# hjr37/diff-gaussian-rasterization

Hardware: AMD Instinct MI355X
Metric: Mviews/sec fwd+bwd @1080p, 500k Gaussians (higher is better)
Workload: dtype f32

## Files before the change

diff-gaussian-rasterization_amd/csrc/dgr_common.h:

```cpp
#pragma once
#include <hip/hip_runtime.h>
#include <stdint.h>

#define DGR_BLOCK_X 16
#define DGR_BLOCK_Y 16
#define DGR_TILE_PIX 256
#define DGR_NEAR 0.2f
#define DGR_TAG_SHIFT 28
#define DGR_ID_MASK ((1u << DGR_TAG_SHIFT) - 1u)
#ifndef DGR_COUNT_STRIDE
#define DGR_COUNT_STRIDE 16
#endif

#define DGR_SCHED_CLASSES 32

namespace dgr {

__host__ __device__ inline size_t align_up(size_t x, size_t a) { return (x + a - 1) / a * a; }

__device__ inline uint32_t sched_class(uint32_t n) {
    if (n == 0u) return 0u;
    const uint32_t l = 31u - (uint32_t)__clz((int)n);
    const uint32_t half = l ? (n >> (l - 1u)) & 1u : 0u;
    const uint32_t c = 1u + 2u * l + half;
    return c < (uint32_t)DGR_SCHED_CLASSES - 1u ? c : (uint32_t)DGR_SCHED_CLASSES - 1u;
}

#ifndef DGR_REC_STRIDE
#define DGR_REC_STRIDE 4
#endif
struct GeometryView {
    float4* rec;
    float* depths;
    int* radii;
    ushort4* rect;
    uint8_t* clamped;
    uint32_t* goff;
    uint32_t* block_tiles;
    float4* shd;
    size_t bytes;
};
__host__ __device__ inline GeometryView carve_geometry(char* base, int P) {
    GeometryView g;
    size_t o = 0;
    g.rec = (float4*)(base + o);      o = align_up(o + sizeof(float4) * DGR_REC_STRIDE * (size_t)P, 256);
    g.depths = (float*)(base + o);    o = align_up(o + sizeof(float) * (size_t)P, 256);
    g.radii = (int*)(base + o);       o = align_up(o + sizeof(int) * (size_t)P, 256);
    g.rect = (ushort4*)(base + o);    o = align_up(o + sizeof(ushort4) * (size_t)P, 256);
    g.clamped = (uint8_t*)(base + o); o = align_up(o + (size_t)P, 256);
    g.goff = (uint32_t*)(base + o);   o = align_up(o + sizeof(uint32_t) * (size_t)P, 256);
    g.block_tiles = (uint32_t*)(base + o); o = align_up(o + sizeof(uint32_t) * (((size_t)P + 255) / 256), 256);
    g.shd = (float4*)(base + o);      o = align_up(o + sizeof(float4) * 3 * (size_t)P, 256);
    g.bytes = o;
    return g;
}

enum { BLEND_SCHEDULE = 1, BLEND_LISTS_QUADRANT = 4, BLEND_LISTS_AUTO = 8 };
enum { BLEND_FLAG_SCHEDULE = 1, BLEND_FLAG_OVERFLOWED = 2, BLEND_FLAG_QUADRANT_LISTS = 4 };

struct ImageView {
    int* status;
    uint32_t* cursor;
    uint32_t* tile_count;
    uint2* ranges;
    uint4* tile_sched;
    uint32_t* n_contrib;
    float* final_T;
    uint32_t* n_valid;
    uint32_t* first_contrib;
    size_t bytes;
};
__host__ __device__ inline int tiles_x(int W) { return (W + DGR_BLOCK_X - 1) / DGR_BLOCK_X; }
__host__ __device__ inline int tiles_y(int H) { return (H + DGR_BLOCK_Y - 1) / DGR_BLOCK_Y; }
__host__ __device__ inline ImageView carve_image(char* base, int W, int H) {
    ImageView v;
    const size_t tiles = (size_t)tiles_x(W) * tiles_y(H), N = (size_t)W * H;
    size_t o = 0;
    v.status = (int*)(base + o);
    v.cursor = (uint32_t*)(base + o + 64);  o = align_up(o + 4 * sizeof(int), 256);
    v.tile_count = (uint32_t*)(base + o); o = align_up(o + tiles * 4 * DGR_COUNT_STRIDE, 256);
    v.ranges = (uint2*)(base + o);        o = align_up(o + tiles * 8, 256);
    v.tile_sched = (uint4*)(base + o);    o = align_up(o + tiles * 16, 256);
    v.n_contrib = (uint32_t*)(base + o);  o = align_up(o + N * 4, 256);
    v.final_T = (float*)(base + o);       o = align_up(o + N * 4, 256);
    v.n_valid = (uint32_t*)(base + o);    o = align_up(o + N * 4, 256);
// ... 113 lines not shown
```

diff-gaussian-rasterization_amd/csrc/gaussian_math.h:

```cpp
#pragma once
#include "dgr_common.h"

#pragma clang fp contract(off)

namespace dgr {
namespace {

struct M3 {
    float m[3][3];
};
__device__ __forceinline__ M3 mul(const M3& A, const M3& B) {
    M3 R;
#pragma unroll
    for (int c = 0; c < 3; c++)
#pragma unroll
        for (int r = 0; r < 3; r++) R.m[c][r] = A.m[0][r] * B.m[c][0] + A.m[1][r] * B.m[c][1] + A.m[2][r] * B.m[c][2];
    return R;
}
__device__ __forceinline__ M3 transpose(const M3& A) {
    M3 R;
#pragma unroll
    for (int c = 0; c < 3; c++)
#pragma unroll
        for (int r = 0; r < 3; r++) R.m[c][r] = A.m[r][c];
// ... 127 lines not shown
    const M3 S = diag3(mod * sc.x, mod * sc.y, mod * sc.z);
    const M3 Mm = mul(S, R);
    const M3 Sigma = mul(transpose(Mm), Mm);
    c3[0] = Sigma.m[0][0]; c3[1] = Sigma.m[0][1]; c3[2] = Sigma.m[0][2];
    c3[3] = Sigma.m[1][1]; c3[4] = Sigma.m[1][2]; c3[5] = Sigma.m[2][2];
}
template <class Args>
__device__ __forceinline__ void load_cov3d(const Args& a, int idx, float (&c3)[6]) {
    if (a.cov3D_precomp) {
        const float* c3p = a.cov3D_precomp + 6 * (size_t)idx;
#pragma unroll
        for (int i = 0; i < 6; i++) c3[i] = c3p[i];
    } else {
        compute_cov3d(a.scales, a.rotations, a.scale_modifier, idx, c3);
    }
}

}

constexpr int SHT_ROWS = 32, SHT_LD = 52;
__device__ __forceinline__ void wave_sync() {
    __builtin_amdgcn_fence(__ATOMIC_ACQ_REL, "wavefront");
    __builtin_amdgcn_wave_barrier();
}
__device__ __forceinline__ void store_streaming(float4* dst, float4 v) {
    typedef float v4f __attribute__((ext_vector_type(4)));
    __builtin_nontemporal_store(v4f{v.x, v.y, v.z, v.w}, reinterpret_cast<v4f*>(dst));
}
__device__ __forceinline__ float4 load_streaming(const float4* src) {
    typedef float v4f __attribute__((ext_vector_type(4)));
    const v4f v = __builtin_nontemporal_load(reinterpret_cast<const v4f*>(src));
    return make_float4(v.x, v.y, v.z, v.w);
}
__device__ __forceinline__ void sh_rows_to_lanes(const float* __restrict__ src, size_t g_block, float* lds, float (&f)[48]) {
    const int wave = threadIdx.x >> 6, lane = threadIdx.x & 63;
    float* my = lds + wave * (SHT_ROWS * SHT_LD);
    const float4* base = reinterpret_cast<const float4*>(src) + (g_block + (size_t)wave * 64) * 12;
#pragma unroll
    for (int r = 0; r < 2; r++) {
        const float4* p = base + (size_t)r * SHT_ROWS * 12;
#pragma unroll
        for (int i = 0; i < 6; i++) {
            const int e = i * 64 + lane;
            const int g = e / 12, c = e - 12 * g;
            *reinterpret_cast<float4*>(my + g * SHT_LD + 4 * c) = load_streaming(p + e);
        }
        wave_sync();
        if ((lane >> 5) == r) {
            const float* row = my + (lane & 31) * SHT_LD;
#pragma unroll
            for (int c = 0; c < 12; c++) {
                const float4 v = *reinterpret_cast<const float4*>(row + 4 * c);
                f[4 * c] = v.x; f[4 * c + 1] = v.y; f[4 * c + 2] = v.z; f[4 * c + 3] = v.w;
            }
        }
        wave_sync();
    }
}
__device__ __forceinline__ void lanes_to_sh_rows(const float (&f)[48], float* __restrict__ dst, size_t g_block, float* lds) {
    const int wave = threadIdx.x >> 6, lane = threadIdx.x & 63;
    float* my = lds + wave * (SHT_ROWS * SHT_LD);
    float4* base = reinterpret_cast<float4*>(dst) + (g_block + (size_t)wave * 64) * 12;
#pragma unroll
    for (int r = 0; r < 2; r++) {
        if ((lane >> 5) == r) {
            float* row = my + (lane & 31) * SHT_LD;
#pragma unroll
            for (int c = 0; c < 12; c++)
                *reinterpret_cast<float4*>(row + 4 * c) = make_float4(f[4 * c], f[4 * c + 1], f[4 * c + 2], f[4 * c + 3]);
        }
        wave_sync();
        float4* p = base + (size_t)r * SHT_ROWS * 12;
#pragma unroll
        for (int i = 0; i < 6; i++) {
            const int e = i * 64 + lane;
            const int g = e / 12, c = e - 12 * g;
            store_streaming(p + e, *reinterpret_cast<const float4*>(my + g * SHT_LD + 4 * c));
        }
        wave_sync();
    }
}
// ... 88 lines not shown
```

diff-gaussian-rasterization_amd/csrc/preprocess_bwd.hip:

```cpp
#include "dgr_common.h"
#include <algorithm>

#include "kernels.h"
#include "gaussian_math.h"
#include "pose_reduce.h"

#pragma clang fp contract(off)
#ifndef DGR_BWD_BATCH_WAVES
#define DGR_BWD_BATCH_WAVES 2
#endif

namespace dgr {

template <bool COMPLETE = false>
__device__ __forceinline__ void bwd_view_terms(const PreprocessBwdArgs& a, const bool full, float3 m, const float (&c3)[6],
                                               const float (&acc)[16], bool vis, uint8_t cl_in, float4 shd0, float4 shd1,
                                               float4 shd2, float3& dmean_out, float (&dcov)[6], float (&coef)[16],
                                               float3& dRGB, float (&pose)[12]) {
    float3 dmean = make_float3(0.f, 0.f, 0.f);
    if (!full) {
        const float* v = a.view;
        const float mul3 = v[2] * m.x + v[6] * m.y + v[10] * m.z + v[14];
        const float med = (COMPLETE && a.map_off) ? 0.0f : acc[10];
        dmean = make_float3((v[2] - v[3] * mul3) * med, (v[6] - v[7] * mul3) * med, (v[10] - v[11] * mul3) * med);
    }
    float3 s_cam = make_float3(0.f, 0.f, 0.f);
    const bool do_map = vis && !a.map_off;
    const bool do_terms = COMPLETE ? vis : do_map;
    float px[12];
    float3 g_cam = make_float3(0.f, 0.f, 0.f);
#pragma unroll
    for (int i = 0; i < 12; i++) px[i] = 0.0f;
#pragma unroll
    for (int i = 0; i < 6; i++) dcov[i] = 0.0f;
    if (do_terms) {
        const float3 dconic = make_float3(acc[6], acc[7], acc[8]);
        Cov2D c;
        cov2d_common(m, a.focal_x, a.focal_y, a.tan_fovx, a.tan_fovy, c3, a.view, c);
        const float limx = 1.3f * a.tan_fovx, limy = 1.3f * a.tan_fovy;
        const float x_grad_mul = (c.txtz < -limx || c.txtz > limx) ? 0.f : 1.f;
        const float y_grad_mul = (c.tytz < -limy || c.tytz > limy) ? 0.f : 1.f;
        const float h_x = a.focal_x, h_y = a.focal_y;
        const M3& T = c.T; const M3& Vrk = c.Vrk; const M3& W = c.W; const float3 t = c.t;
        const float ca = c.cov.m[0][0] + 0.3f, cb = c.cov.m[0][1], cc = c.cov.m[1][1] + 0.3f;
        const float denom = ca * cc - cb * cb;
        float dL_da = 0, dL_db = 0, dL_dc = 0;
        const float denom2inv = 1.0f / ((denom * denom) + 0.0000001f);
        if (denom2inv != 0) {
            dL_da = denom2inv * (-cc * cc * dconic.x + 2 * cb * cc * dconic.y + (denom - ca * cc) * dconic.z);
            dL_dc = denom2inv * (-ca * ca * dconic.z + 2 * ca * cb * dconic.y + (denom - ca * cc) * dconic.x);
// ... 63 lines not shown
        const float4 m_hom = xform4x4(m, pj);
        const float m_w = 1.0f / (m_hom.w + 0.0000001f);
        const float mul1 = (pj[0] * m.x + pj[4] * m.y + pj[8] * m.z + pj[12]) * m_w * m_w;
        const float mul2 = (pj[1] * m.x + pj[5] * m.y + pj[9] * m.z + pj[13]) * m_w * m_w;
        const float g2x = acc[4], g2y = acc[5];
        float3 d1;
        d1.x = (pj[0] * m_w - pj[3] * mul1) * g2x + (pj[1] * m_w - pj[3] * mul2) * g2y;
        d1.y = (pj[4] * m_w - pj[7] * mul1) * g2x + (pj[5] * m_w - pj[7] * mul2) * g2y;
        d1.z = (pj[8] * m_w - pj[11] * mul1) * g2x + (pj[9] * m_w - pj[11] * mul2) * g2y;
        if (!COMPLETE || do_map) { dmean.x += d1.x; dmean.y += d1.y; dmean.z += d1.z; }
        if (!full && (!COMPLETE || do_map)) {
            const float mul3 = v[2] * m.x + v[6] * m.y + v[10] * m.z + v[14];
            float3 d2;
            d2.x = (v[2] - v[3] * mul3) * acc[3];
            d2.y = (v[6] - v[7] * mul3) * acc[3];
            d2.z = (v[10] - v[11] * mul3) * acc[3];
            dmean.x += d2.x; dmean.y += d2.y; dmean.z += d2.z;
        }
    }
#pragma unroll
    for (int k = 0; k < 16; k++) coef[k] = 0.0f;
    dRGB = make_float3(0.f, 0.f, 0.f);
    const bool sh_out = a.dL_dsh && do_map;
    if ((COMPLETE ? true : a.dL_dsh != nullptr) && a.M > 0 && do_terms && a.shs) {
        const float3 cam = make_float3(a.campos[0], a.campos[1], a.campos[2]);
        const float3 dir_orig = m - cam;
        const float len = sqrtf(dot3(dir_orig, dir_orig));
        const float3 dir = make_float3(dir_orig.x / len, dir_orig.y / len, dir_orig.z / len);
        const uint8_t cl = cl_in;
        dRGB = make_float3(acc[0], acc[1], acc[2]);
        dRGB.x *= (cl & 1) ? 0 : 1;
        dRGB.y *= (cl & 2) ? 0 : 1;
        dRGB.z *= (cl & 4) ? 0 : 1;
        const float3 dRGBdx = make_float3(shd0.x, shd0.y, shd0.z), dRGBdy = make_float3(shd1.x, shd1.y, shd1.z),
                     dRGBdz = make_float3(shd2.x, shd2.y, shd2.z);
        const float x = dir.x, y = dir.y, z = dir.z;
        coef[0] = SH_C0;
        if (a.D > 0) {
            coef[1] = -SH_C1 * y;
            coef[2] = SH_C1 * z;
            coef[3] = -SH_C1 * x;
            if (a.D > 1) {
                const float xx = x * x, yy = y * y, zz = z * z, xy = x * y, yz = y * z, xz = x * z;
                coef[4] = SH_C2[0] * xy;
                coef[5] = SH_C2[1] * yz;
                coef[6] = SH_C2[2] * (2.f * zz - xx - yy);
                coef[7] = SH_C2[3] * xz;
                coef[8] = SH_C2[4] * (xx - yy);
                if (a.D > 2) {
                    coef[9] = SH_C3[0] * y * (3.f * xx - yy);
                    coef[10] = SH_C3[1] * xy * z;
                    coef[11] = SH_C3[2] * y * (4.f * zz - xx - yy);
                    coef[12] = SH_C3[3] * z * (2.f * zz - 3.f * xx - 3.f * yy);
                    coef[13] = SH_C3[4] * x * (4.f * zz - xx - yy);
                    coef[14] = SH_C3[5] * z * (xx - yy);
                    coef[15] = SH_C3[6] * x * (xx - 3.f * yy);
                }
            }
        }
        if (full) {
            const float len3 = len * len * len;
            const float i3 = 1.0f / len3, i1 = 1.0f / len;
            const float3 o = dir_orig;
            const float3 raw = make_float3(acc[0], acc[1], acc[2]);
            const float3 cx = dRGBdx * (o.x * o.x * i3 - i1) + dRGBdy * (o.x * o.y * i3) + dRGBdz * (o.x * o.z * i3);
            const float3 cy = dRGBdx * (o.x * o.y * i3) + dRGBdy * (o.y * o.y * i3 - i1) + dRGBdz * (o.y * o.z * i3);
            const float3 cz = dRGBdx * (o.x * o.z * i3) + dRGBdy * (o.y * o.z * i3) + dRGBdz * (o.z * o.z * i3 - i1);
            s_cam = make_float3(dot3(raw, cx), dot3(raw, cy), dot3(raw, cz));
// ... 102 lines not shown
#endif
template <bool COMPLETE>
__global__ void __launch_bounds__(256, DGR_PPB_WAVES) preprocess_bwd_kernel(PreprocessBwdArgs a) {
    const int idx = blockIdx.x * 256 + threadIdx.x;
    float pose[12];
#pragma unroll
    for (int i = 0; i < 12; i++) pose[i] = 0.0f;

    if (idx < a.P) {
        float4* ap = reinterpret_cast<float4*>(a.acc + (size_t)idx * DGR_ACC_STRIDE);
        const float4 a0 = ap[0], a1 = ap[1], a2 = ap[2], a3 = ap[3];
        const int rad = a.radii[idx];

        const float3 m = load_row3(a.means3D, idx);
        const bool need_map = !a.map_off;
        const bool need_terms = COMPLETE || need_map;
        float c3[6] = {0.f, 0.f, 0.f, 0.f, 0.f, 0.f};
        if (need_terms) {
            if (a.cov3D_precomp) {
                const float* c3p = a.cov3D_precomp + 6 * (size_t)idx;
#pragma unroll
                for (int i = 0; i < 6; i++) c3[i] = c3p[i];
            } else {
                compute_cov3d(a.scales, a.rotations, a.scale_modifier, idx, c3);
            }
        }
        float3 sc_in = make_float3(0.f, 0.f, 0.f);
        float4 q_in = make_float4(0.f, 0.f, 0.f, 0.f);
        if (need_map && a.scales) {
            sc_in = load_row3(a.scales, idx);
            q_in = load_row4(a.rotations, idx);
        }
        uint8_t cl_in = 0;
        float4 shd0 = make_float4(0.f, 0.f, 0.f, 0.f), shd1 = shd0, shd2 = shd0;
        if (need_terms) {
            cl_in = a.geom.clamped[idx];
            shd0 = a.geom.shd[idx]; shd1 = a.geom.shd[(size_t)a.P + idx]; shd2 = a.geom.shd[2 * (size_t)a.P + idx];
        }
        const bool vis = rad > 0;
        float acc[16];
        unpack_acc_row(a0, a1, a2, a3, vis, acc);

        write_dmean2D(a, idx, acc);
        const bool zero_copies = COMPLETE && a.map_off;
        if (a.dL_dopacity) a.dL_dopacity[idx] = zero_copies ? 0.0f : acc[9];
        if (a.dL_dcolor) {
            a.dL_dcolor[3 * (size_t)idx + 0] = zero_copies ? 0.0f : acc[0];
            a.dL_dcolor[3 * (size_t)idx + 1] = zero_copies ? 0.0f : acc[1];
            a.dL_dcolor[3 * (size_t)idx + 2] = zero_copies ? 0.0f : acc[2];
        }
        if (a.dL_ddepth) a.dL_ddepth[idx] = zero_copies ? 0.0f : acc[3];
        if (a.dL_dconic) {
            float4* o = reinterpret_cast<float4*>(a.dL_dconic) + idx;
            *o = zero_copies ? make_float4(0.0f, 0.0f, 0.0f, 0.0f) : make_float4(acc[6], acc[7], 0.0f, acc[8]);
        }

        float3 dmean;
        float dcov[6], coef[16];
        float3 dRGB;
        bwd_view_terms<COMPLETE>(a, a.full_variant != 0, m, c3, acc, vis, cl_in, shd0, shd1, shd2, dmean, dcov, coef, dRGB, pose);
        float3 dscale = make_float3(0, 0, 0);
        float4 drot = make_float4(0, 0, 0, 0);
        const bool do_map = vis && !a.map_off;
        const int ncoef_out = a.M;

        if (a.dL_dsh && ncoef_out > 0) {
            float3* out = reinterpret_cast<float3*>(a.dL_dsh) + (size_t)idx * ncoef_out;
            __shared__ float sht[4 * SHT_ROWS * SHT_LD];
            const bool blk_fast = a.sh_vec_ok && ncoef_out == 16 && a.shs != nullptr && (size_t)blockIdx.x * 256 + 256 <= (size_t)a.P;
            if (do_map && a.shs) {
                if (blk_fast) {
                } else if (a.sh_vec_ok && ncoef_out == 16) {
                    const float ch[3] = {dRGB.x, dRGB.y, dRGB.z};
                    float4* o4 = reinterpret_cast<float4*>(out);
#pragma unroll
                    for (int i = 0; i < 12; i++)
                        o4[i] = make_float4(coef[(4 * i) / 3] * ch[(4 * i) % 3], coef[(4 * i + 1) / 3] * ch[(4 * i + 1) % 3],
                                            coef[(4 * i + 2) / 3] * ch[(4 * i + 2) % 3], coef[(4 * i + 3) / 3] * ch[(4 * i + 3) % 3]);
                } else {
#pragma unroll
                    for (int k = 0; k < 16; k++)
                        if (k < ncoef_out) out[k] = coef[k] * dRGB;
                }
            } else if (!blk_fast) {
                if (a.sh_vec_ok && ncoef_out == 16) {
                    float4* o4 = reinterpret_cast<float4*>(out);
#pragma unroll
                    for (int i = 0; i < 12; i++) o4[i] = make_float4(0, 0, 0, 0);
                } else {
                    for (int k = 0; k < ncoef_out; k++) out[k] = make_float3(0, 0, 0);
                }
            }
            if (blk_fast) lanes_to_sh_rows_scaled(coef, dRGB, a.dL_dsh, (size_t)blockIdx.x * 256, sht);
// ... 41 lines not shown
    const int P = b.base.P, V = b.V;
    const bool in = idx < P;
    __shared__ float sht[4 * SHT_ROWS * SHT_LD];
    __shared__ double red[DGR_MAX_BATCH_VIEWS][16][12];
    float3 m = make_float3(0.f, 0.f, 0.f), sc_in = make_float3(0.f, 0.f, 0.f);
    float4 q_in = make_float4(0.f, 0.f, 0.f, 0.f);
    float c3[6] = {0.f, 0.f, 0.f, 0.f, 0.f, 0.f};
    if (in) {
        m = load_row3(b.base.means3D, idx);
        if (b.base.cov3D_precomp || b.base.scales) load_cov3d(b.base, idx, c3);
        if (b.base.scales) {
            sc_in = load_row3(b.base.scales, idx);
            q_in = load_row4(b.base.rotations, idx);
        }
    }
    float3 dmean_s = make_float3(0.f, 0.f, 0.f), dcol_s = make_float3(0.f, 0.f, 0.f);
    float dcov_s[6] = {0.f, 0.f, 0.f, 0.f, 0.f, 0.f};
    float dop_s = 0.0f;
    float dsh[48];
#pragma unroll
    for (int e = 0; e < 48; e++) dsh[e] = 0.0f;
    bool any_map = false;
#pragma unroll 1
    for (int v = 0; v < V; v++) {
        const PreprocessBwdArgs a = batch_view_args(b, v);
        float pose[12];
#pragma unroll
        for (int i = 0; i < 12; i++) pose[i] = 0.0f;
        if (in) {
            const float4* ap = reinterpret_cast<const float4*>(a.acc + (size_t)idx * DGR_ACC_STRIDE);
            const float4 a0 = ap[0], a1 = ap[1], a2 = ap[2], a3 = ap[3];
            const int rad = a.radii[idx];
            const uint8_t cl_in = a.geom.clamped[idx];
            const float4 shd0 = a.geom.shd[idx], shd1 = a.geom.shd[(size_t)P + idx], shd2 = a.geom.shd[2 * (size_t)P + idx];
            const bool vis = rad > 0;
            float acc[16];
            unpack_acc_row(a0, a1, a2, a3, vis, acc);
            write_dmean2D(a, idx, acc);
            float3 dmean, dRGB;
            float dcov[6], coef[16];
            bwd_view_terms<COMPLETE>(a, FULL, m, c3, acc, vis, cl_in, shd0, shd1, shd2, dmean, dcov, coef, dRGB, pose);
            any_map |= vis && !a.map_off;
            if (!(COMPLETE && a.map_off)) {
                dop_s += acc[9];
                dcol_s.x += acc[0]; dcol_s.y += acc[1]; dcol_s.z += acc[2];
            }
            dmean_s.x += dmean.x; dmean_s.y += dmean.y; dmean_s.z += dmean.z;
#pragma unroll
            for (int i = 0; i < 6; i++) dcov_s[i] += dcov[i];
            const float ch[3] = {dRGB.x, dRGB.y, dRGB.z};
#pragma unroll
            for (int e = 0; e < 48; e++) dsh[e] += coef[e / 3] * ch[e % 3];
        }
        if (a.track_off) {
            pose_zero(a.dL_dview);
        } else {
            pose_rows_to_lds(pose, red[v]);
        }
    }
    const int M = b.base.M;
    const bool blk_fast = b.base.dL_dsh && b.base.sh_vec_ok && M == 16 && (size_t)blockIdx.x * 256 + 256 <= (size_t)P;
    if (in) {
        float3 dscale = make_float3(0, 0, 0);
        float4 drot = make_float4(0, 0, 0, 0);
        if (any_map && b.base.scales) cov3d_backward_terms(sc_in, q_in, b.base.scale_modifier, dcov_s, dscale, drot);
        if (b.base.dL_dopacity) b.base.dL_dopacity[idx] = dop_s;
        if (b.base.dL_dcolor) store_row3(b.base.dL_dcolor, idx, dcol_s);
        if (b.base.dL_dmean3D) store_row3(b.base.dL_dmean3D, idx, dmean_s);
        if (b.base.dL_dcov3D) store_row6(b.base.dL_dcov3D, idx, dcov_s);
        if (b.base.dL_dscale) store_row3(b.base.dL_dscale, idx, dscale);
        if (b.base.dL_drot) store_row4(b.base.dL_drot, idx, drot);
        if (b.base.dL_dsh && M > 0 && !blk_fast) {
            float* out = b.base.dL_dsh + (size_t)idx * M * 3;
#pragma unroll
// ... 65 lines not shown
```

diff-gaussian-rasterization_amd/csrc/preprocess_fwd.hip:

```cpp
#include "dgr_common.h"

#include "kernels.h"
#include "count_rank.h"
#include "gaussian_math.h"

#pragma clang fp contract(off)

namespace dgr {

struct FwdGeom {
    int radius;
    ushort4 rect;
    bool violation, need_sh;
};
template <bool C3_GIVEN>
__device__ __forceinline__ FwdGeom fwd_view_geometry(const PreprocessFwdArgs& a, int idx, float3 p_orig, const float (&c3_in)[6]) {
    int radius = 0;
    ushort4 rect = make_ushort4(0, 0, 0, 0);
    bool violation = false, need_sh = false;
    if (a.gau_uncertainty) a.gau_uncertainty[idx] = 0.0f;
    if (a.gau_related_pixels) a.gau_related_pixels[idx] = 0;
    const float4 p_hom = xform4x4(p_orig, a.proj);
    const float p_w = 1.0f / (p_hom.w + 0.0000001f);
    const float3 p_proj = make_float3(p_hom.x * p_w, p_hom.y * p_w, p_hom.z * p_w);
// ... 62 lines not shown
    if (a.radii_out) a.radii_out[idx] = radius;
    a.geom.rect[idx] = rect;
    return FwdGeom{radius, rect, violation, need_sh};
}

__device__ __forceinline__ void fwd_view_colour(const PreprocessFwdArgs& a, int idx, float3 p_orig, const SHCoeffs& s) {
    float3 rgb;
    const float3 cam = make_float3(a.campos[0], a.campos[1], a.campos[2]);
    float3 dir = p_orig - cam;
    const float len = sqrtf(dot3(dir, dir));
    dir = make_float3(dir.x / len, dir.y / len, dir.z / len);
    float3 res = SH_C0 * s.c[0];
    if (a.D > 0) {
        const float x = dir.x, y = dir.y, z = dir.z;
        res = res - SH_C1 * y * s.c[1] + SH_C1 * z * s.c[2] - SH_C1 * x * s.c[3];
        if (a.D > 1) {
            const float xx = x * x, yy = y * y, zz = z * z, xy = x * y, yz = y * z, xz = x * z;
            res = res + SH_C2[0] * xy * s.c[4] + SH_C2[1] * yz * s.c[5] +
                  SH_C2[2] * (2.0f * zz - xx - yy) * s.c[6] + SH_C2[3] * xz * s.c[7] +
                  SH_C2[4] * (xx - yy) * s.c[8];
            if (a.D > 2) {
                res = res + SH_C3[0] * y * (3.0f * xx - yy) * s.c[9] + SH_C3[1] * xy * z * s.c[10] +
                      SH_C3[2] * y * (4.0f * zz - xx - yy) * s.c[11] +
                      SH_C3[3] * z * (2.0f * zz - 3.0f * xx - 3.0f * yy) * s.c[12] +
                      SH_C3[4] * x * (4.0f * zz - xx - yy) * s.c[13] +
                      SH_C3[5] * z * (xx - yy) * s.c[14] + SH_C3[6] * x * (xx - 3.0f * yy) * s.c[15];
            }
        }
    }
    res.x += 0.5f; res.y += 0.5f; res.z += 0.5f;
    {
        float3 dRGBdx = make_float3(0, 0, 0), dRGBdy = make_float3(0, 0, 0), dRGBdz = make_float3(0, 0, 0);
        sh_direction_derivatives(s, a.D, dir, dRGBdx, dRGBdy, dRGBdz);
        float4* shd = a.geom.shd + (size_t)idx;
        shd[0] = make_float4(dRGBdx.x, dRGBdx.y, dRGBdx.z, 0.0f);
        shd[(size_t)a.P] = make_float4(dRGBdy.x, dRGBdy.y, dRGBdy.z, 0.0f);
        shd[2 * (size_t)a.P] = make_float4(dRGBdz.x, dRGBdz.y, dRGBdz.z, 0.0f);
    }
    a.geom.clamped[idx] = (uint8_t)((res.x < 0 ? 1 : 0) | (res.y < 0 ? 2 : 0) | (res.z < 0 ? 4 : 0));
    rgb = make_float3(fmaxf(res.x, 0.0f), fmaxf(res.y, 0.0f), fmaxf(res.z, 0.0f));
    a.geom.rec[DGR_REC_STRIDE * (size_t)idx + 2] = make_float4(rgb.x, rgb.y, rgb.z, 0.0f);
}

__device__ __forceinline__ void fetch_sh(const PreprocessFwdArgs& a, int idx, bool need, float* lds, SHCoeffs& s) {
    const bool blk_fast = a.sh_vec_ok && a.M == 16 && (size_t)blockIdx.x * 256 + 256 <= (size_t)a.P && __syncthreads_or(need);
    float shf[48];
    if (blk_fast) sh_rows_to_lanes(a.shs, (size_t)blockIdx.x * 256, lds, shf);
    if (need) {
        if (blk_fast) {
#pragma unroll
            for (int k = 0; k < 16; k++) s.c[k] = make_float3(shf[3 * k], shf[3 * k + 1], shf[3 * k + 2]);
        } else {
            load_sh(a.shs, idx, a.D, a.M, a.sh_vec_ok, s);
        }
    }
}

__device__ __forceinline__ uint32_t wave_tiles_word(ushort4 rect, bool violation) {
    uint32_t n = (uint32_t)(rect.z - rect.x) * (uint32_t)(rect.w - rect.y);
#pragma unroll
    for (int off = 32; off > 0; off >>= 1) n += __shfl_xor(n, off, 64);
    if (__builtin_amdgcn_ballot_w64(violation) != 0ull) n |= 0x80000000u;
    return n;
}
__device__ __forceinline__ uint32_t block_tiles_word(const uint32_t* w) {
    const uint32_t flag = (w[0] | w[1] | w[2] | w[3]) & 0x80000000u;
    return ((w[0] & 0x7fffffffu) + (w[1] & 0x7fffffffu) + (w[2] & 0x7fffffffu) + (w[3] & 0x7fffffffu)) | flag;
}

__device__ __forceinline__ uint32_t block_exclusive_scan4(uint32_t n, uint32_t* wtot , int tid, uint32_t* total) {
    const int lane = tid & 63, wave = tid >> 6;
    uint32_t incl = n;
#pragma unroll
    for (int off = 1; off < 64; off <<= 1) {
        const uint32_t v = __shfl_up(incl, off, 64);
        if (lane >= off) incl += v;
    }
    if (lane == 63) wtot[wave] = incl;
    __syncthreads();
    uint32_t before = 0;
// ... 135 lines not shown
```

diff-gaussian-rasterization_amd/csrc/torch_ext.cpp:

```cpp
#include <torch/extension.h>

#include <ATen/hip/impl/HIPGuardImplMasqueradingAsCUDA.h>
#include <ATen/hip/impl/HIPStreamMasqueradingAsCUDA.h>
#include <ATen/hip/impl/HIPCachingAllocatorMasqueradingAsCUDA.h>

#include <array>
#include <tuple>

#include "torch_support.h"

namespace {

using namespace dgr_ext;
using torch::autograd::AutogradContext;
using torch::autograd::variable_list;

inline Tensor f32c(const Tensor& t, const c10::Device& dev) {
    if (t.numel() == 0 || (t.scalar_type() == at::kFloat && t.is_contiguous() && t.device() == dev)) return t;
    return t.to(dev, at::kFloat).contiguous();
}
inline Tensor f32c_diag4(const Tensor& t, const c10::Device& dev) {
    if (t.scalar_type() == at::kFloat && t.device() == dev && t.dim() == 2 && t.size(0) == 4 && t.size(1) == 4 && t.stride(0) == 1 &&
        t.stride(1) == 4 && ((dgr_thread_options_effective() >> DGR_OPT_SHIFT_POSE_GRAD) & 15) != 2)
        return t;
// ... 91 lines not shown
            run(cap);
        } catch (...) {
            int unused[4];
            if (ticket >= 0) (void)dgr_status_poll(ticket, 1, unused);
            throw;
        }
        o.cap = cap;
        if (mode == 2) {
            o.ticket = ticket;
            return;
        }
        int s[4] = {0, 0, 0, 0};
        check(dgr_status_poll(ticket, 1, s));
        if (s[2]) throw std::runtime_error("Point is filtered although prefiltered is set. This shouldn't happen!");
        o.rendered = s[0];
        if (o.rendered <= cap) return;
        cap = (long)(o.rendered * 1.1) + 4096;
    }
}

struct AbsGrad {
    Tensor t;
    float* view[DGR_MAX_BATCH_VIEWS] = {};
    AbsGrad(bool on, const Tensor& means3D, long V) {
        if (!on) return;
        const long P = means3D.size(0);
        const auto f32 = at::TensorOptions().dtype(at::kFloat).device(means3D.device());
        t = V ? at::empty({V, P, 3}, f32) : at::empty({P, 3}, f32);
        for (long v = 0; v < std::max(V, 1L) && v < DGR_MAX_BATCH_VIEWS && P > 0; v++) view[v] = row<float>(t, v);
    }
    float* const* views() const { return t.defined() ? view : nullptr; }
};

inline void grad_arena(const c10::Device& dev, int P, int M, Tensor* g, float** gp) {
    carve(dev, {{&g[3], {P, 3}, at::kFloat}, {&g[0], {P, 3}, at::kFloat}, {&g[5], {P, M, 3}, at::kFloat}, {&g[2], {P, 1}, at::kFloat},
                {&g[6], {P, 3}, at::kFloat}, {&g[7], {P, 4}, at::kFloat}, {&g[4], {P, 6}, at::kFloat}, {&g[1], {P, 3}, at::kFloat}});
    for (int i = 0; i < 8; i++) gp[i] = ptr<float>(g[i]);
}

struct BwdScene {
    c10::Device dev;
    c10::hip::HIPGuardMasqueradingAsCUDA guard;
    int P, M, degree;
    float scale_modifier, tan_fovx, tan_fovy;
    Tensor means3D, bg, colors, scales, rotations, cov3D, view, proj, campos, gt, sh, perspec;
    const Tensor &radii, &geom, &binning, &img, &perspec_arg;
    BwdScene(const Tensor& background, const Tensor& means3D_, const Tensor& radii_, const Tensor& colors_, const Tensor& scales_,
             const Tensor& rotations_, double scale_modifier_, const Tensor& cov3D_, const Tensor& view_, const Tensor& proj_,
             double tan_fovx_, double tan_fovy_, const Tensor& gt_, const Tensor& sh_, long degree_, const Tensor& campos_,
             const Tensor& geom_, const Tensor& binning_, const Tensor& img_, const Tensor& perspec_)
        : dev(means3D_.device()), guard(dev), P((int)means3D_.size(0)), degree((int)degree_), scale_modifier((float)scale_modifier_),
          tan_fovx((float)tan_fovx_), tan_fovy((float)tan_fovy_), means3D(f32c(means3D_, dev)), bg(f32c(background, dev)),
          colors(f32c(colors_, dev)), scales(f32c(scales_, dev)), rotations(f32c(rotations_, dev)), cov3D(f32c(cov3D_, dev)),
          view(f32c(view_, dev)), proj(f32c(proj_, dev)), campos(f32c(campos_, dev)), gt(f32c(gt_, dev)), sh(f32c(sh_, dev)),
          perspec(f32c_diag4(perspec_, dev)), radii(radii_), geom(geom_), binning(binning_), img(img_), perspec_arg(perspec_) {
        M = sh.numel() != 0 ? (int)sh.size(1) : 0;
    }
};
struct BwdFlags {
    bool debug = false, track_off = false, map_off = false;
};

struct BatchBwdOut {
    std::vector<Tensor> g = std::vector<Tensor>(9);
    float* gp[8] = {nullptr, nullptr, nullptr, nullptr, nullptr, nullptr, nullptr, nullptr};
    Tensor scratch;
    size_t nscr;
    BatchBwdOut(const c10::Device& dev, int P, int M, long V, long W, long H, bool need_gaussian_grads, bool need_means2D,
                const std::vector<long>& num_rendered) {
        const auto f32 = at::TensorOptions().dtype(at::kFloat).device(dev);
// ... 209 lines not shown
        Alloc3 al{{&o.geom, dev}, {&o.binning, dev}, {&o.img, dev}};
        const int rc = V::forward(std::tuple_cat(std::make_tuple(st, cb_geom, cb_binning, cb_img, &al), args), debug, o.related);
        check(rc);
        o.rendered = o.cap = rc;
        return o;
    }
    auto run = [&](long cap) {
        Probe p_st(HP_STATE_ALLOC);
        const StateArena sa(dev, P, (int)W, (int)H, cap);
        o.geom = sa.geom; o.binning = sa.binning; o.img = sa.img;
        p_st.stop();
        Probe p_c(HP_FWD_C);
        check(V::forward_presized(std::tuple_cat(std::make_tuple(st, (char*)o.geom.data_ptr(), (char*)o.binning.data_ptr(), (int)cap,
                                                                 (char*)o.img.data_ptr(), o.status.data_ptr<int>()), args)));
    };
    presized_forward(run, capacity, mode, st, o);
    if (mode != 2) V::after_strict(o, st, debug, want_related);
    return o;
}

template <class V>
PyForward forward(const Tensor& background, const Tensor& means3D, const Tensor& colors, const Tensor& opacity, const Tensor& scales,
                  const Tensor& rotations, double scale_modifier, const Tensor& cov3D, const Tensor& viewmatrix, const Tensor& gt_depth,
                  const Tensor& projmatrix, double tan_fovx, double tan_fovy, long H, long W, const Tensor& sh, long degree,
                  const Tensor& campos, bool prefiltered, bool debug, long capacity, long mode) {
    const Fwd o = forward_core<V>(background, means3D, colors, opacity, scales, rotations, scale_modifier, cov3D, viewmatrix, gt_depth,
                                  projmatrix, tan_fovx, tan_fovy, H, W, sh, degree, campos, prefiltered, debug, capacity, mode,
                                  true);
    return {o.py(), V::forward_tensors(o)};
}

template <class V>
std::vector<Tensor> backward(const BwdScene& s, const std::array<const Tensor*, V::N_IMAGES>& images, long R, BwdFlags flags,
                             bool need_gaussian_grads, bool absgrad) {
    AbsGrad abs(absgrad, s.means3D, 0);
    const c10::Device dev = s.dev;
    const long H = images[V::GC]->size(1), W = images[V::GC]->size(2);
    typename V::Images im;
    for (size_t i = 0; i < im.size(); i++) im[i] = f32c(*images[i], dev);
    const Tensor* recorded[V::N_IMAGES + 1];
    *std::copy(images.begin(), images.end(), recorded) = &s.perspec_arg;
    keep_until_read(dev, recorded, std::size(recorded));
    Probe p_al(HP_BWD_ALLOC);
    std::vector<Tensor> g(9);
    float* gp[8] = {nullptr, nullptr, nullptr, nullptr, nullptr, nullptr, nullptr, nullptr};
    if (need_gaussian_grads) grad_arena(dev, s.P, s.M, g.data(), gp);
    const size_t nscr = up256(dgr_light_backward_scratch_bytes_r(s.P, (int)W, (int)H, (int)R));
    void* st = stream_of(dev);
    const auto f32 = at::TensorOptions().dtype(at::kFloat).device(dev);
    g[8] = V::dview_leading_one ? at::empty({1, 4, 4}, f32) : at::empty({4, 4}, f32);
    on_backward_scratch(dev, st, nscr, [&](char* scratch) {
        p_al.stop();
        Probe p_bc(HP_BWD_C);
        return V::backward(st, s, im, W, H, R, gp, g[8].data_ptr<float>(), flags, need_gaussian_grads, scratch, nscr, abs.view[0]);
    });
    if (absgrad) g.push_back(std::move(abs.t));
    return g;
}

std::vector<Tensor> light_backward(const Tensor& background, const Tensor& means3D, const Tensor& radii, const Tensor& colors,
                                   const Tensor& scales, const Tensor& rotations, double scale_modifier, const Tensor& cov3D,
                                   const Tensor& viewmatrix, const Tensor& projmatrix, double tan_fovx, double tan_fovy,
                                   const Tensor& dL_dout_color, const Tensor& dL_dout_depth, const Tensor& dL_dout_median,
                                   const Tensor& dL_dout_var, const Tensor& gt_depth, const Tensor& sh, long degree, const Tensor& campos,
                                   const Tensor& geomBuffer, long R, const Tensor& binningBuffer, const Tensor& imageBuffer,
                                   const Tensor& alphas, bool debug, const Tensor& perspec, bool track_off, bool map_off,
                                   bool need_gaussian_grads, const Tensor& dL_dout_alpha, bool absgrad) {
    const BwdScene s(background, means3D, radii, colors, scales, rotations, scale_modifier, cov3D, viewmatrix, projmatrix, tan_fovx,
                     tan_fovy, gt_depth, sh, degree, campos, geomBuffer, binningBuffer, imageBuffer, perspec);
    return backward<Light>(s, {&dL_dout_color, &dL_dout_depth, &dL_dout_median, &dL_dout_var, &dL_dout_alpha, &alphas}, R,
                           {debug, track_off, map_off}, need_gaussian_grads, absgrad);
}
std::vector<Tensor> full_backward(const Tensor& background, const Tensor& means3D, const Tensor& radii, const Tensor& colors,
                                  const Tensor& scales, const Tensor& rotations, double scale_modifier, const Tensor& cov3D,
                                  const Tensor& viewmatrix, const Tensor& gt_depth, const Tensor& projmatrix, double tan_fovx,
                                  double tan_fovy, const Tensor& dL_dout_color, const Tensor& dL_dout_depth, const Tensor& dL_dout_unc,
                                  const Tensor& sh, long degree, const Tensor& campos, const Tensor& geomBuffer, long R,
                                  const Tensor& binningBuffer, const Tensor& imageBuffer, long NG, const Tensor& perspec,
                                  bool need_gaussian_grads, const Tensor& dL_dout_sil, bool absgrad) {
// ... 90 lines not shown
                                      capacity, mode, false);
        g_report = o;
        Probe p_s(HP_SAVE);
        variable_list sv(V::N_SAVED);
        sv[S_COLORS] = colors_precomp; sv[S_MEANS3D] = means3D; sv[S_SCALES] = scales; sv[S_ROTATIONS] = rotations;
        sv[S_COV3D] = cov3Ds_precomp; sv[S_VIEW] = viewmatrix; sv[S_RADII] = o.radii; sv[S_SH] = sh; sv[S_GEOM] = o.geom;
        sv[S_BINNING] = o.binning; sv[S_IMG] = o.img; sv[S_GT] = gt_depth; sv[S_BG] = bg; sv[S_PROJ] = projmatrix;
        sv[S_CAMPOS] = campos; sv[S_PERSPEC] = perspec;
        V::save_extra(sv, o);
        ctx->save_for_backward(std::move(sv));
        SavedScalars{scale_modifier, tanfovx, tanfovy, degree, (int64_t)(o.rendered >= 0 ? o.rendered : o.cap), H, W,
                     (int64_t)dgr_thread_options_effective(), track_off, map_off}
            .write(ctx->saved_data, V::tracking_flags);
        ctx->set_materialize_grads(false);
        ctx->mark_non_differentiable(V::non_differentiable(o));
        return V::node_outputs(o);
    }

    static variable_list backward(AutogradContext* ctx, variable_list grad) {
        Probe p_b(HP_BWD);
        Probe p_u(HP_UNPACK);
        const auto sv = ctx->get_saved_variables();
        SavedScalars c;
        c.read(ctx->saved_data, V::tracking_flags);
        const Tensor& means3D = sv[S_MEANS3D];
        const c10::Device dev = means3D.device();
        p_u.stop();
        const Tensor gC = grad_or_zeros(grad[0], 3, c.H, c.W, dev), gD = grad_or_zeros(grad[2], 1, c.H, c.W, dev), none;
        const auto images = V::node_images(gC, gD, grad, sv, silhouette_on((int)c.options), none);
        const UnderOptions under((int)c.options);
        const BwdScene s(sv[S_BG], means3D, sv[S_RADII], sv[S_COLORS], sv[S_SCALES], sv[S_ROTATIONS], c.scale_modifier, sv[S_COV3D],
                         sv[S_VIEW], sv[S_PROJ], c.tanfovx, c.tanfovy, sv[S_GT], sv[S_SH], c.degree, sv[S_CAMPOS], sv[S_GEOM],
                         sv[S_BINNING], sv[S_IMG], sv[S_PERSPEC]);
        std::vector<Tensor> g = ::backward<V>(s, images, c.R, {false, c.track_off, c.map_off}, needs_gaussian_grads(ctx), false);
        consume_post_backward_wait(stream_of(dev));
        if (V::dview_leading_one) g[8] = view_of(g[8], 0, {4, 4}, at::kFloat);
        return node_grads(g);
    }
};

template <class V>
PyForward apply(const Tensor& means3D, const Tensor& means2D, const Tensor& sh, const Tensor& colors_precomp, const Tensor& opacities,
                const Tensor& scales, const Tensor& rotations, const Tensor& cov3Ds_precomp, const Tensor& viewmatrix,
                const Tensor& gt_depth, const Tensor& bg, const Tensor& projmatrix, const Tensor& campos, const Tensor& perspec,
                double scale_modifier, double tanfovx, double tanfovy, long H, long W, long degree, bool prefiltered, bool track_off,
                bool map_off, long capacity, long mode) {
    Probe p_a(HP_APPLY);
    variable_list out = Node<V>::apply(means3D, means2D, sh, colors_precomp, opacities, scales, rotations, cov3Ds_precomp, viewmatrix,
                                       gt_depth, bg, projmatrix, campos, perspec, scale_modifier, tanfovx, tanfovy, (int64_t)H,
                                       (int64_t)W, (int64_t)degree, prefiltered, track_off, map_off, (int64_t)capacity, (int64_t)mode);
    p_a.stop();
    PyForward result{g_report.py(), std::move(out)};
    g_report.status = Tensor();
    return result;
}

inline long batch_size(long V) {
    if (V < 1 || V > DGR_MAX_BATCH_VIEWS) throw std::runtime_error("1 .. " + std::to_string(DGR_MAX_BATCH_VIEWS) + " views per batch");
    return V;
}
std::vector<long> post_batch_status(bool post_status, int P, void* st, const Tensor& status, long V) {
    std::vector<long> tickets;
    if (post_status && P > 0 && !dgr_stream_is_capturing(st)) {
        for (long v = 0; v < V; v++) {
            const long t = dgr_status_post(st, row<int>(status, v));
            check(t);
            tickets.push_back(t);
// ... 124 lines not shown
```

diff-gaussian-rasterization_amd/dgr_amd/_frontend.py:

```python
import ctypes as C
import os
import threading
from typing import NamedTuple

import torch

from . import _binning, _capi
from ._binning import _check

MAX_VIEWS = _capi.MAX_BATCH_VIEWS
_row = _capi.row_ptr

ext = None
if os.environ.get("DGR_BINDING", "compiled") != "ctypes" and not os.environ.get("DGR_HIP_LIB"):
    try:
        from . import _dgr_torch_ext as ext
    except ImportError:
        pass


def _ext():
    from . import light
    return ext if light._C is light._CompiledC else None

# ... 415 lines not shown
    ctx.raster_settings = raster_settings
    ctx.num_rendered = R
    ctx.absgrad = means2D_abs is not None
    ctx.dgr_options = _capi.load().dgr_thread_options_effective()
    ctx.silhouette = _capi.silhouette_on(ctx.dgr_options)
    ctx.save_for_backward(colors_precomp, means3D, scales, rotations, cov3Ds_precomp, viewmatrix, radii, sh, geom, binning, img,
                          *[results[i] for i in saved], gt_depth)
    ctx.set_materialize_grads(False)
    ctx.mark_non_differentiable(*[results[i] for i in non_differentiable])
    return tuple([results[i] for i in returns])


def _run_backward(ctx, variant, batch, grad_outputs, call):
    saved = ctx.saved_tensors
    absgrad = ctx.absgrad
    null = None if batch else _EMPTY
    silhouette = grad_outputs[variant.silhouette_slot] if ctx.silhouette else None
    images = []
    for slot, channels, *rules in variant.image_slots:
        image = grad_outputs[slot]
        if ctx.silhouette and slot == variant.silhouette_slot:
            image = null
        elif image is None:
            rule = rules[batch]
            if rule is ZEROS or (rule is LEAN_WITH_ABSGRAD and not absgrad):
                rs = ctx.raster_settings
                image = torch.zeros(((saved[5].size(0),) if batch else ()) + (channels, int(rs.image_height), int(rs.image_width)),
                                    dtype=torch.float32, device=saved[1].device)
            else:
                image = null
        images.append(image)
    with _capi.under_options(ctx.dgr_options):
        out = call(saved, images, absgrad or any(ctx.needs_input_grad[:8]), silhouette)
    (grad_means2D, grad_colors_precomp, grad_opacities, grad_means3D, grad_cov3Ds_precomp, grad_sh, grad_scales, grad_rotations,
     grad_viewmatrix) = out[:9]
    _consume_post_backward_wait()
    return (grad_means3D, grad_means2D, grad_sh, grad_colors_precomp, grad_opacities, grad_scales, grad_rotations,
            grad_cov3Ds_precomp, grad_viewmatrix, None, None, out[9] if absgrad else None)
```

Measured before the change: 0.002769.

## Pack SH derivative cache, skip unneeded SH loads, and drop unused grad buffers

The SH direction derivatives are stored as two float4 arrays plus one float array, 9 floats in place of 12 padded ones, which cuts forward writes and backward reads. The block-fast SH transpose now takes a ballot mask and skips global loads for Gaussians that do not need SH evaluation. The gradient arena stops allocating colors_precomp and cov3D gradients when they are not required, and the Python frontend nulls them. The backward batch-wave count also goes from 2 to 3, and the extra live registers in the masked loads could lower occupancy.

```diff
diff --git a/diff-gaussian-rasterization_amd/csrc/dgr_common.h b/diff-gaussian-rasterization_amd/csrc/dgr_common.h
--- a/diff-gaussian-rasterization_amd/csrc/dgr_common.h
+++ b/diff-gaussian-rasterization_amd/csrc/dgr_common.h
@@ -37,7 +37,9 @@
     uint8_t* clamped;
     uint32_t* goff;
     uint32_t* block_tiles;
-    float4* shd;
+    float4* shd_a;
+    float4* shd_b;
+    float* shd_c;
     size_t bytes;
 };
 __host__ __device__ inline GeometryView carve_geometry(char* base, int P) {
@@ -50,7 +52,11 @@
     g.clamped = (uint8_t*)(base + o); o = align_up(o + (size_t)P, 256);
     g.goff = (uint32_t*)(base + o);   o = align_up(o + sizeof(uint32_t) * (size_t)P, 256);
     g.block_tiles = (uint32_t*)(base + o); o = align_up(o + sizeof(uint32_t) * (((size_t)P + 255) / 256), 256);
-    g.shd = (float4*)(base + o);      o = align_up(o + sizeof(float4) * 3 * (size_t)P, 256);
+    const size_t shd_region_end = align_up(o + sizeof(float4) * 3 * (size_t)P, 256);
+    g.shd_a = (float4*)(base + o);    o = align_up(o + sizeof(float4) * (size_t)P, 256);
+    g.shd_b = (float4*)(base + o);    o = align_up(o + sizeof(float4) * (size_t)P, 256);
+    g.shd_c = (float*)(base + o);     o = align_up(o + sizeof(float) * (size_t)P, 256);
+    if (o < shd_region_end) o = shd_region_end;
     g.bytes = o;
     return g;
 }
diff --git a/diff-gaussian-rasterization_amd/csrc/gaussian_math.h b/diff-gaussian-rasterization_amd/csrc/gaussian_math.h
--- a/diff-gaussian-rasterization_amd/csrc/gaussian_math.h
+++ b/diff-gaussian-rasterization_amd/csrc/gaussian_math.h
@@ -183,21 +183,30 @@
     const v4f v = __builtin_nontemporal_load(reinterpret_cast<const v4f*>(src));
     return make_float4(v.x, v.y, v.z, v.w);
 }
-__device__ __forceinline__ void sh_rows_to_lanes(const float* __restrict__ src, size_t g_block, float* lds, float (&f)[48]) {
+__device__ __forceinline__ void sh_rows_to_lanes(const float* __restrict__ src, size_t g_block, float* lds, uint64_t need, float (&f)[48]) {
     const int wave = threadIdx.x >> 6, lane = threadIdx.x & 63;
     float* my = lds + wave * (SHT_ROWS * SHT_LD);
     const float4* base = reinterpret_cast<const float4*>(src) + (g_block + (size_t)wave * 64) * 12;
 #pragma unroll
     for (int r = 0; r < 2; r++) {
+        const uint32_t slab_need = (uint32_t)(need >> (32 * r));
+        if (slab_need == 0u) continue;
         const float4* p = base + (size_t)r * SHT_ROWS * 12;
+        float4 v[6];
+#pragma unroll
+        for (int i = 0; i < 6; i++) {
+            const int e = i * 64 + lane;
+            v[i] = make_float4(0.f, 0.f, 0.f, 0.f);
+            if ((slab_need >> (e / 12)) & 1u) v[i] = load_streaming(p + e);
+        }
 #pragma unroll
         for (int i = 0; i < 6; i++) {
             const int e = i * 64 + lane;
             const int g = e / 12, c = e - 12 * g;
-            *reinterpret_cast<float4*>(my + g * SHT_LD + 4 * c) = load_streaming(p + e);
-        }
-        wave_sync();
-        if ((lane >> 5) == r) {
+            *reinterpret_cast<float4*>(my + g * SHT_LD + 4 * c) = v[i];
+        }
+        wave_sync();
+        if ((lane >> 5) == r && ((slab_need >> (lane & 31)) & 1u)) {
             const float* row = my + (lane & 31) * SHT_LD;
 #pragma unroll
             for (int c = 0; c < 12; c++) {
diff --git a/diff-gaussian-rasterization_amd/csrc/preprocess_bwd.hip b/diff-gaussian-rasterization_amd/csrc/preprocess_bwd.hip
--- a/diff-gaussian-rasterization_amd/csrc/preprocess_bwd.hip
+++ b/diff-gaussian-rasterization_amd/csrc/preprocess_bwd.hip
@@ -7,15 +7,15 @@
 
 #pragma clang fp contract(off)
 #ifndef DGR_BWD_BATCH_WAVES
-#define DGR_BWD_BATCH_WAVES 2
+#define DGR_BWD_BATCH_WAVES 3
 #endif
 
 namespace dgr {
 
 template <bool COMPLETE = false>
 __device__ __forceinline__ void bwd_view_terms(const PreprocessBwdArgs& a, const bool full, float3 m, const float (&c3)[6],
-                                               const float (&acc)[16], bool vis, uint8_t cl_in, float4 shd0, float4 shd1,
-                                               float4 shd2, float3& dmean_out, float (&dcov)[6], float (&coef)[16],
+                                               const float (&acc)[16], bool vis, uint8_t cl_in, float4 shd_a, float4 shd_b,
+                                               float shd_c, float3& dmean_out, float (&dcov)[6], float (&coef)[16],
                                                float3& dRGB, float (&pose)[12]) {
     float3 dmean = make_float3(0.f, 0.f, 0.f);
     if (!full) {
@@ -145,8 +145,8 @@
         dRGB.x *= (cl & 1) ? 0 : 1;
         dRGB.y *= (cl & 2) ? 0 : 1;
         dRGB.z *= (cl & 4) ? 0 : 1;
-        const float3 dRGBdx = make_float3(shd0.x, shd0.y, shd0.z), dRGBdy = make_float3(shd1.x, shd1.y, shd1.z),
-                     dRGBdz = make_float3(shd2.x, shd2.y, shd2.z);
+        const float3 dRGBdx = make_float3(shd_a.x, shd_a.y, shd_a.z), dRGBdy = make_float3(shd_a.w, shd_b.x, shd_b.y),
+                     dRGBdz = make_float3(shd_b.z, shd_b.w, shd_c);
         const float x = dir.x, y = dir.y, z = dir.z;
         coef[0] = SH_C0;
         if (a.D > 0) {
@@ -315,10 +315,11 @@
             q_in = load_row4(a.rotations, idx);
         }
         uint8_t cl_in = 0;
-        float4 shd0 = make_float4(0.f, 0.f, 0.f, 0.f), shd1 = shd0, shd2 = shd0;
+        float4 shd_a = make_float4(0.f, 0.f, 0.f, 0.f), shd_b = shd_a;
+        float shd_c = 0.f;
         if (need_terms) {
             cl_in = a.geom.clamped[idx];
-            shd0 = a.geom.shd[idx]; shd1 = a.geom.shd[(size_t)a.P + idx]; shd2 = a.geom.shd[2 * (size_t)a.P + idx];
+            shd_a = a.geom.shd_a[idx]; shd_b = a.geom.shd_b[idx]; shd_c = a.geom.shd_c[idx];
         }
         const bool vis = rad > 0;
         float acc[16];
@@ -341,7 +342,7 @@
         float3 dmean;
         float dcov[6], coef[16];
         float3 dRGB;
-        bwd_view_terms<COMPLETE>(a, a.full_variant != 0, m, c3, acc, vis, cl_in, shd0, shd1, shd2, dmean, dcov, coef, dRGB, pose);
+        bwd_view_terms<COMPLETE>(a, a.full_variant != 0, m, c3, acc, vis, cl_in, shd_a, shd_b, shd_c, dmean, dcov, coef, dRGB, pose);
         float3 dscale = make_float3(0, 0, 0);
         float4 drot = make_float4(0, 0, 0, 0);
         const bool do_map = vis && !a.map_off;
@@ -449,14 +450,15 @@
             const float4 a0 = ap[0], a1 = ap[1], a2 = ap[2], a3 = ap[3];
             const int rad = a.radii[idx];
             const uint8_t cl_in = a.geom.clamped[idx];
-            const float4 shd0 = a.geom.shd[idx], shd1 = a.geom.shd[(size_t)P + idx], shd2 = a.geom.shd[2 * (size_t)P + idx];
+            const float4 shd_a = a.geom.shd_a[idx], shd_b = a.geom.shd_b[idx];
+            const float shd_c = a.geom.shd_c[idx];
             const bool vis = rad > 0;
             float acc[16];
             unpack_acc_row(a0, a1, a2, a3, vis, acc);
             write_dmean2D(a, idx, acc);
             float3 dmean, dRGB;
             float dcov[6], coef[16];
-            bwd_view_terms<COMPLETE>(a, FULL, m, c3, acc, vis, cl_in, shd0, shd1, shd2, dmean, dcov, coef, dRGB, pose);
+            bwd_view_terms<COMPLETE>(a, FULL, m, c3, acc, vis, cl_in, shd_a, shd_b, shd_c, dmean, dcov, coef, dRGB, pose);
             any_map |= vis && !a.map_off;
             if (!(COMPLETE && a.map_off)) {
                 dop_s += acc[9];
diff --git a/diff-gaussian-rasterization_amd/csrc/preprocess_fwd.hip b/diff-gaussian-rasterization_amd/csrc/preprocess_fwd.hip
--- a/diff-gaussian-rasterization_amd/csrc/preprocess_fwd.hip
+++ b/diff-gaussian-rasterization_amd/csrc/preprocess_fwd.hip
@@ -118,10 +118,9 @@
     {
         float3 dRGBdx = make_float3(0, 0, 0), dRGBdy = make_float3(0, 0, 0), dRGBdz = make_float3(0, 0, 0);
         sh_direction_derivatives(s, a.D, dir, dRGBdx, dRGBdy, dRGBdz);
-        float4* shd = a.geom.shd + (size_t)idx;
-        shd[0] = make_float4(dRGBdx.x, dRGBdx.y, dRGBdx.z, 0.0f);
-        shd[(size_t)a.P] = make_float4(dRGBdy.x, dRGBdy.y, dRGBdy.z, 0.0f);
-        shd[2 * (size_t)a.P] = make_float4(dRGBdz.x, dRGBdz.y, dRGBdz.z, 0.0f);
+        a.geom.shd_a[idx] = make_float4(dRGBdx.x, dRGBdx.y, dRGBdx.z, dRGBdy.x);
+        a.geom.shd_b[idx] = make_float4(dRGBdy.y, dRGBdy.z, dRGBdz.x, dRGBdz.y);
+        a.geom.shd_c[idx] = dRGBdz.z;
     }
     a.geom.clamped[idx] = (uint8_t)((res.x < 0 ? 1 : 0) | (res.y < 0 ? 2 : 0) | (res.z < 0 ? 4 : 0));
     rgb = make_float3(fmaxf(res.x, 0.0f), fmaxf(res.y, 0.0f), fmaxf(res.z, 0.0f));
@@ -131,7 +130,7 @@
 __device__ __forceinline__ void fetch_sh(const PreprocessFwdArgs& a, int idx, bool need, float* lds, SHCoeffs& s) {
     const bool blk_fast = a.sh_vec_ok && a.M == 16 && (size_t)blockIdx.x * 256 + 256 <= (size_t)a.P && __syncthreads_or(need);
     float shf[48];
-    if (blk_fast) sh_rows_to_lanes(a.shs, (size_t)blockIdx.x * 256, lds, shf);
+    if (blk_fast) sh_rows_to_lanes(a.shs, (size_t)blockIdx.x * 256, lds, __builtin_amdgcn_ballot_w64(need), shf);
     if (need) {
         if (blk_fast) {
 #pragma unroll
diff --git a/diff-gaussian-rasterization_amd/csrc/torch_ext.cpp b/diff-gaussian-rasterization_amd/csrc/torch_ext.cpp
--- a/diff-gaussian-rasterization_amd/csrc/torch_ext.cpp
+++ b/diff-gaussian-rasterization_amd/csrc/torch_ext.cpp
@@ -147,10 +147,15 @@
     float* const* views() const { return t.defined() ? view : nullptr; }
 };
 
-inline void grad_arena(const c10::Device& dev, int P, int M, Tensor* g, float** gp) {
-    carve(dev, {{&g[3], {P, 3}, at::kFloat}, {&g[0], {P, 3}, at::kFloat}, {&g[5], {P, M, 3}, at::kFloat}, {&g[2], {P, 1}, at::kFloat},
-                {&g[6], {P, 3}, at::kFloat}, {&g[7], {P, 4}, at::kFloat}, {&g[4], {P, 6}, at::kFloat}, {&g[1], {P, 3}, at::kFloat}});
-    for (int i = 0; i < 8; i++) gp[i] = ptr<float>(g[i]);
+inline void grad_arena(const c10::Device& dev, int P, int M, Tensor* g, float** gp, bool want_colors = true, bool want_cov3D = true) {
+    const int64_t s3[] = {P, 3}, ssh[] = {P, M, 3}, s1[] = {P, 1}, s4[] = {P, 4}, s6[] = {P, 6};
+    const Window w[8] = {{&g[3], s3, at::kFloat}, {&g[0], s3, at::kFloat}, {&g[5], ssh, at::kFloat}, {&g[2], s1, at::kFloat},
+                         {&g[6], s3, at::kFloat}, {&g[7], s4, at::kFloat}, {&g[4], s6, at::kFloat}, {&g[1], s3, at::kFloat}};
+    if (want_colors && want_cov3D) carve(dev, {w[0], w[1], w[2], w[3], w[4], w[5], w[6], w[7]});
+    else if (want_cov3D) carve(dev, {w[0], w[1], w[2], w[3], w[4], w[5], w[6]});
+    else if (want_colors) carve(dev, {w[0], w[1], w[2], w[3], w[4], w[5], w[7]});
+    else carve(dev, {w[0], w[1], w[2], w[3], w[4], w[5]});
+    for (int i = 0; i < 8; i++) gp[i] = g[i].defined() ? ptr<float>(g[i]) : nullptr;
 }
 
 struct BwdScene {
@@ -426,7 +431,7 @@
 
 template <class V>
 std::vector<Tensor> backward(const BwdScene& s, const std::array<const Tensor*, V::N_IMAGES>& images, long R, BwdFlags flags,
-                             bool need_gaussian_grads, bool absgrad) {
+                             bool need_gaussian_grads, bool absgrad, bool want_colors = true, bool want_cov3D = true) {
     AbsGrad abs(absgrad, s.means3D, 0);
     const c10::Device dev = s.dev;
     const long H = images[V::GC]->size(1), W = images[V::GC]->size(2);
@@ -438,7 +443,7 @@
     Probe p_al(HP_BWD_ALLOC);
     std::vector<Tensor> g(9);
     float* gp[8] = {nullptr, nullptr, nullptr, nullptr, nullptr, nullptr, nullptr, nullptr};
-    if (need_gaussian_grads) grad_arena(dev, s.P, s.M, g.data(), gp);
+    if (need_gaussian_grads) grad_arena(dev, s.P, s.M, g.data(), gp, want_colors, want_cov3D);
     const size_t nscr = up256(dgr_light_backward_scratch_bytes_r(s.P, (int)W, (int)H, (int)R));
     void* st = stream_of(dev);
     const auto f32 = at::TensorOptions().dtype(at::kFloat).device(dev);
@@ -595,7 +600,10 @@
         const BwdScene s(sv[S_BG], means3D, sv[S_RADII], sv[S_COLORS], sv[S_SCALES], sv[S_ROTATIONS], c.scale_modifier, sv[S_COV3D],
                          sv[S_VIEW], sv[S_PROJ], c.tanfovx, c.tanfovy, sv[S_GT], sv[S_SH], c.degree, sv[S_CAMPOS], sv[S_GEOM],
                          sv[S_BINNING], sv[S_IMG], sv[S_PERSPEC]);
-        std::vector<Tensor> g = ::backward<V>(s, images, c.R, {false, c.track_off, c.map_off}, needs_gaussian_grads(ctx), false);
+        const bool want_colors = ctx->needs_input_grad(3) && sv[S_COLORS].numel() != 0;
+        const bool want_cov3D = ctx->needs_input_grad(7) && sv[S_COV3D].numel() != 0;
+        std::vector<Tensor> g = ::backward<V>(s, images, c.R, {false, c.track_off, c.map_off}, needs_gaussian_grads(ctx), false,
+                                              want_colors, want_cov3D);
         consume_post_backward_wait(stream_of(dev));
         if (V::dview_leading_one) g[8] = view_of(g[8], 0, {4, 4}, at::kFloat);
         return node_grads(g);
diff --git a/diff-gaussian-rasterization_amd/dgr_amd/_frontend.py b/diff-gaussian-rasterization_amd/dgr_amd/_frontend.py
--- a/diff-gaussian-rasterization_amd/dgr_amd/_frontend.py
+++ b/diff-gaussian-rasterization_amd/dgr_amd/_frontend.py
@@ -471,6 +471,10 @@
         images.append(image)
     with _capi.under_options(ctx.dgr_options):
         out = call(saved, images, absgrad or any(ctx.needs_input_grad[:8]), silhouette)
+    if not batch:
+        keep = {1: ctx.needs_input_grad[3] and saved[0] is not None and saved[0].numel() != 0,
+                4: ctx.needs_input_grad[7] and saved[4] is not None and saved[4].numel() != 0}
+        out = tuple(x if keep.get(i, True) else None for i, x in enumerate(out))
     (grad_means2D, grad_colors_precomp, grad_opacities, grad_means3D, grad_cov3Ds_precomp, grad_sh, grad_scales, grad_rotations,
      grad_viewmatrix) = out[:9]
     _consume_post_backward_wait()
```

Result: faster. 0.002833 (median of 6 runs) (+2.3%).
